# pandegroup/openmm

Hardware: NVIDIA H100
Metric: ns/day (higher is better)
Workload: dtype f32

## Files before the change

openmm_b200/csrc/engine.cu:

```cuda
#include "engine.h"
#include "../../include/b200md.h"
#include <stdexcept>
#include <algorithm>
#include <cmath>
#include <cstring>
#include <cstdlib>
#include <map>
#include <set>
#include <dlfcn.h>
#include <thread>

static std::string g_create_error;

template <class T> struct DevBuf {
    T* p = nullptr; size_t n = 0; bool owned = true;
    void attach(void* ptr, size_t count) { free(); p = (T*) ptr; n = count; owned = false; }
    void alloc(size_t count) {
        if (!owned) { if (count > n) throw std::runtime_error("window buffer too small"); return; }
        free(); n = count; if (count) CUDA_CHECK(cudaMalloc(&p, count*sizeof(T)));
    }
    void upload(const std::vector<T>& v) { if (v.size() > n) alloc(v.size()); if (!v.empty()) CUDA_CHECK(cudaMemcpy(p, v.data(), v.size()*sizeof(T), cudaMemcpyHostToDevice)); }
    void zero() { if (n) CUDA_CHECK(cudaMemset(p, 0, n*sizeof(T))); }
    void free() { if (p && owned) cudaFree(p); p = nullptr; n = 0; owned = true; }
    ~DevBuf() { free(); }
// ... 5 lines not shown
    void* lib = nullptr;
    int (*GetUniqueId)(void*) = nullptr;
    int (*CommInitRank)(void**, int, NcclUid, int) = nullptr;
    int (*AllReduce)(const void*, void*, size_t, int, int, void*, cudaStream_t) = nullptr;
    int (*AllGather)(const void*, void*, size_t, int, void*, cudaStream_t) = nullptr;
    int (*CommDestroy)(void*) = nullptr;
    const char* (*GetErrorString)(int) = nullptr;
    bool load(std::string& err) {
        if (lib) return true;
        const char* names[] = {getenv("B200MD_NCCL_LIB"), "libnccl.so.2", "libnccl.so"};
        for (const char* nm : names) { if (nm && (lib = dlopen(nm, RTLD_NOW | RTLD_GLOBAL))) break; }
        if (!lib) { err = "cannot dlopen libnccl (set B200MD_NCCL_LIB)"; return false; }
        GetUniqueId = (decltype(GetUniqueId)) dlsym(lib, "ncclGetUniqueId");
        CommInitRank = (decltype(CommInitRank)) dlsym(lib, "ncclCommInitRank");
        AllReduce = (decltype(AllReduce)) dlsym(lib, "ncclAllReduce");
        AllGather = (decltype(AllGather)) dlsym(lib, "ncclAllGather");
        CommDestroy = (decltype(CommDestroy)) dlsym(lib, "ncclCommDestroy");
        GetErrorString = (decltype(GetErrorString)) dlsym(lib, "ncclGetErrorString");
        if (!GetUniqueId || !CommInitRank || !AllReduce) { err = "libnccl lacks required symbols"; return false; }
        return true;
    }
};
static NcclApi g_nccl;
enum { NCCL_INT8 = 0, NCCL_INT64 = 4, NCCL_FLOAT32 = 7, NCCL_FLOAT64 = 8, NCCL_SUM = 0 };

struct b200md_ctx {
    int device = 0;
    int natoms = 0, npad = 0, nblocks = 0;
    bool finalized = false;
    std::string err;
    cudaStream_t stream = nullptr;
    cudaStream_t streamPme = nullptr;
    cudaStream_t streamBonded = nullptr;
    cudaEvent_t evFork = nullptr, evJoin = nullptr, evJoinBonded = nullptr;
    bool pmeOnly = false;
    bool listDirty = true;
    bool overlapPme = true;
    bool pmeBrick = true;
    int brickAtoms = 64, brickPoints = 8192;
    bool listBuilt = false;
    std::vector<double> mass, charge, sigma, epsilon;
    b200md_nonbonded_desc nbdesc{};
    bool haveNb = false;
    std::vector<int> excI, excJ; std::vector<double> excQQ, excSig, excEps;
    std::vector<int> bondI, bondJ; std::vector<double> bondR0, bondK;
    std::vector<int> angI, angJ, angK; std::vector<double> angT0, angKK;
    std::vector<int> torI, torJ, torK, torL, torN; std::vector<double> torPhase, torKK;
    std::vector<int> rbI, rbJ, rbK, rbL; std::vector<double> rbC;
    std::vector<int> cmapSize, cmapMap, cmapAtoms; std::vector<double> cmapCoeff;
    std::vector<unsigned char> bondGroup, angGroup, torGroup, rbGroup, cmapGroup;
    std::vector<int> conI, conJ; std::vector<double> conD;
    int cmFreq = 0;
    std::vector<int4> hUnitAtoms;
    double boxA[3] = {0, 0, 0}, boxB[3] = {0, 0, 0}, boxC[3] = {0, 0, 0};
    bool haveBox = false;
    bool haveOrigin = false;
    double padFrac = 0.10;
    DevBuf<float4> posq, velm, sposq[2], swrap[2], refPos, atomShift, blockCenter[2], blockHalf[2], superCenter[2], superHalf[2];
    DevBuf<float2> sigeps, ssigeps[2];
    DevBuf<double> chargeD; DevBuf<double2> sigepsD;
    DevBuf<long long> force;
    DevBuf<double> energy, cmScratch;
    DevBuf<int> molStart, molAtoms, cellOffset, sorig[2], sortedOf, cellRank, cellCount, cellFill, atomCell, tmpSorted, tileI[2], tileJ[2], tileMask[2], listCounters, counters, exclStart, exclList;
    DevBuf<unsigned int> maskPool[2];
    DevBuf<unsigned long long> stepCounter;
    DevBuf<unsigned int> blocksDone;
    bool stepStateValid = false;
// ... 58 lines not shown
static void require(bool cond, const char* msg) { if (!cond) throw std::runtime_error(msg); }
static void check_flags(b200md_ctx* c);
static void sync_velocities(b200md_ctx* c);
static void sync_positions(b200md_ctx* c);

extern "C" const char* b200md_version(void) { return "b200md 0.2 (sm_90a)"; }
extern "C" const char* b200md_last_error(const b200md_ctx* ctx) { return ctx ? ctx->err.c_str() : g_create_error.c_str(); }

extern "C" int b200md_create(b200md_ctx** out, int device, int natoms) {
    try {
        require(out != nullptr && natoms > 0, "b200md_create: bad arguments");
        int count = 0;
        cudaError_t e = cudaGetDeviceCount(&count);
        if (e != cudaSuccess || count == 0)
            throw std::runtime_error(std::string("b200md_create: no CUDA device available (") + cudaGetErrorString(e) + "); this library has no CPU fallback");
        require(device >= 0 && device < count, "b200md_create: device index out of range");
        CUDA_CHECK(cudaSetDevice(device));
        b200md_ctx* c = new b200md_ctx();
        c->device = device;
        c->natoms = natoms;
        c->npad = ((natoms + 31)/32)*32;
        c->nblocks = c->npad/32;
        CUDA_CHECK(cudaStreamCreateWithFlags(&c->stream, cudaStreamNonBlocking));
        if (getenv("B200MD_NO_OVERLAP")) c->overlapPme = false;
        if (getenv("B200MD_PME_BRICK")) c->pmeBrick = atoi(getenv("B200MD_PME_BRICK")) != 0;
        if (getenv("B200MD_PME_BRICK_POINTS")) c->brickPoints = std::max(1, atoi(getenv("B200MD_PME_BRICK_POINTS")));
        int hi = 0;
        CUDA_CHECK(cudaDeviceGetStreamPriorityRange(nullptr, &hi));
        CUDA_CHECK(cudaStreamCreateWithPriority(&c->streamPme, cudaStreamNonBlocking, hi));
        CUDA_CHECK(cudaStreamCreateWithPriority(&c->streamBonded, cudaStreamNonBlocking, hi));
        CUDA_CHECK(cudaEventCreateWithFlags(&c->evFork, cudaEventDisableTiming));
        CUDA_CHECK(cudaEventCreateWithFlags(&c->evJoin, cudaEventDisableTiming));
        CUDA_CHECK(cudaEventCreateWithFlags(&c->evJoinBonded, cudaEventDisableTiming));
        c->mass.assign(natoms, 1.0);
        c->charge.assign(natoms, 0.0); c->sigma.assign(natoms, 1.0); c->epsilon.assign(natoms, 0.0);
        const char* pf = getenv("B200MD_PAD_FRACTION");
        if (pf) c->padFrac = atof(pf);
        const char* ug = getenv("B200MD_USE_GRAPH");
        if (ug) c->useGraph = atoi(ug) != 0;
        const char* gs = getenv("B200MD_GRAPH_STEPS");
        if (gs) c->graphSteps = std::max(1, atoi(gs));
        *out = c;
        return 0;
    } catch (std::exception& e) { g_create_error = e.what(); return -1; }
}

extern "C" void b200md_destroy(b200md_ctx* ctx) {
    if (!ctx) return;
    cudaSetDevice(ctx->device);
    cudaDeviceSynchronize();
    if (ctx->stepGraph) cudaGraphExecDestroy(ctx->stepGraph);
    if (ctx->multiGraph) cudaGraphExecDestroy(ctx->multiGraph);
    for (int q = 0; q < B200MD_MAX_RANKS; q++) if (ctx->peerMapped[q]) cudaIpcCloseMemHandle(ctx->peerMapped[q]);
    if (ctx->comm && g_nccl.CommDestroy) g_nccl.CommDestroy(ctx->comm);
    if (ctx->stream) cudaStreamDestroy(ctx->stream);
    if (ctx->streamPme) cudaStreamDestroy(ctx->streamPme);
    if (ctx->streamBonded) cudaStreamDestroy(ctx->streamBonded);
    if (ctx->evFork) cudaEventDestroy(ctx->evFork);
    if (ctx->evJoin) cudaEventDestroy(ctx->evJoin);
    if (ctx->evJoinBonded) cudaEventDestroy(ctx->evJoinBonded);
    char* window = ctx->window;
    delete ctx;
    if (window) cudaFree(window);
}

extern "C" int b200md_set_masses(b200md_ctx* ctx, const double* mass) {
    API_BEGIN(ctx)
    require(!ctx->finalized, "set_masses after finalize");
    ctx->mass.assign(mass, mass + ctx->natoms);
    API_END(ctx)
}

extern "C" int b200md_set_nonbonded(b200md_ctx* ctx, const b200md_nonbonded_desc* d, const double* q, const double* sig, const double* eps) {
    API_BEGIN(ctx)
    require(!ctx->finalized, "set_nonbonded after finalize");
    require(d->method != B200MD_NB_EWALD && d->method != B200MD_NB_LJPME, "nonbonded method not supported by the B200 platform (only NoCutoff, CutoffNonPeriodic, CutoffPeriodic, PME)");
    ctx->nbdesc = *d;
    ctx->haveNb = true;
    ctx->charge.assign(q, q + ctx->natoms);
    ctx->sigma.assign(sig, sig + ctx->natoms);
    ctx->epsilon.assign(eps, eps + ctx->natoms);
    ctx->dispersionCoefficient = d->dispersion_coefficient;
    API_END(ctx)
}

extern "C" int b200md_set_exceptions(b200md_ctx* ctx, int n, const int* p1, const int* p2, const double* qq, const double* sig, const double* eps) {
    API_BEGIN(ctx)
    require(!ctx->finalized, "set_exceptions after finalize");
    ctx->excI.assign(p1, p1+n); ctx->excJ.assign(p2, p2+n);
    ctx->excQQ.assign(qq, qq+n); ctx->excSig.assign(sig, sig+n); ctx->excEps.assign(eps, eps+n);
    API_END(ctx)
}
extern "C" int b200md_set_bonds(b200md_ctx* ctx, int n, const int* p1, const int* p2, const double* len, const double* k) {
// ... 1206 lines not shown
    PmeDev p = c->pme;
    p.brickAtoms = (c->pmeBrick && c->world == 1 && !c->pmeOnly && c->listBuilt) ? c->brickAtoms : 0;
    p.brickPoints = c->brickPoints;
    return p;
}

static int enqueue_forces(b200md_ctx* c, int terms, bool energy, bool forcesAlreadyZero = false, bool inStep = false, unsigned int groupMask = 0xffffffffu) {
    int launches = 0;
    cudaStream_t s = c->stream;
    if (!forcesAlreadyZero) CUDA_CHECK(cudaMemsetAsync(c->force.p, 0, sizeof(long long)*3*c->npad, s));
    if (energy) CUDA_CHECK(cudaMemsetAsync(c->energy.p, 0, sizeof(double)*B200MD_NUM_ENERGY, s));
    bool direct = (terms & B200MD_TERM_NB_DIRECT) && c->haveNb;
    bool recip = (terms & B200MD_TERM_NB_RECIP) && c->haveNb && c->nb.method == B200MD_NB_PME;
    const bool split = role_split(c);
    const int pmeRank = c->world - 1;
    NbDev nbSave = c->nb;
    if (split) {
        if (c->rank == pmeRank) direct = false; else recip = false;
        c->nb = role_nb(c);
    }
    struct Restore { b200md_ctx* c; NbDev saved; ~Restore() { c->nb = saved; } } restore{c, nbSave};
    const bool p2p = c->p2p;
    const bool fork = direct && recip && c->overlapPme && !(c->world > 1 && c->comm && !p2p);
    cudaStream_t sp = fork ? c->streamPme : s;
    if (p2p && !direct) { launch_pos_wait(c->nb, c->cd, s); launches++; }
    const PmeDev pme = pme_for_launch(c);
    const bool forkAfterList = fork && direct && pme.brickAtoms > 0;
    auto launch_recip = [&]() {
        if (fork) {
            CUDA_CHECK(cudaEventRecord(c->evFork, s));
            CUDA_CHECK(cudaStreamWaitEvent(sp, c->evFork, 0));
        }
        if (recip) {
            launch_pme_spread(c->nb, pme, c->cd, sp); launches++;
            if (p2p) { launch_grid_push(c->pme, c->cd, sp); launches++; }
            else if (c->world > 1 && c->comm && !split) {
                int rc = g_nccl.AllReduce(c->gridFixed.p, c->gridFixed.p, (size_t) c->pme.nx*c->pme.ny*c->pme.nz, NCCL_INT64, NCCL_SUM, c->comm, sp);
                if (rc != 0) throw std::runtime_error("ncclAllReduce(grid) failed");
            }
            launch_pme_fft_conv(c->nb, c->pme, c->cd, energy && (split || p2p || c->rank == 0), fft_beside_tiles(c), sp); launches += pme_fft_launch_count(c->pme);
            launch_pme_gather(c->nb, pme, c->cd, sp); launches++;
        }
        if (fork) CUDA_CHECK(cudaEventRecord(c->evJoin, sp));
    };
    if (!forkAfterList) launch_recip();
    if (direct) {
        launch_check_displacement(c->nb, c->cd, s); launches++;
        launch_list_build(c->nb, s); launches += LIST_BUILD_LAUNCHES;
    }
    int bterms = terms & (B200MD_TERM_BONDS | B200MD_TERM_ANGLES | B200MD_TERM_TORSIONS | B200MD_TERM_RB_TORSIONS | B200MD_TERM_CMAP);
    if (c->haveNb) bterms |= terms & B200MD_TERM_NB_DIRECT;
    const int nbonded = c->bd.nbonds + c->bd.nangles + c->bd.ntorsions + c->bd.nrb + c->bd.ncmap + c->bd.nexc;
    const bool bonded = bterms && nbonded > 0 && !(split && c->rank == pmeRank);
    auto launch_bonded_terms = [&](cudaStream_t sb) { BondedDev bd = c->bd; bd.groupMask = groupMask; launch_bonded(c->nb, bd, bterms, energy, sb); launches++; };
    const bool forkBonded = forkAfterList && bonded;
    if (forkAfterList) launch_recip();
    if (forkBonded) {
        CUDA_CHECK(cudaStreamWaitEvent(c->streamBonded, c->evFork, 0));
        launch_bonded_terms(c->streamBonded);
        CUDA_CHECK(cudaEventRecord(c->evJoinBonded, c->streamBonded));
    }
    if (direct) { launch_pair(c->nb, energy, s); launches++; }
    if (bonded && !forkBonded) launch_bonded_terms(s);
    const bool pushEarly = p2p && fork;
    if (pushEarly) { launch_force_push(c->nb, c->cd, s); launches++; }
    if (fork) CUDA_CHECK(cudaStreamWaitEvent(s, c->evJoin, 0));
    if (forkBonded) CUDA_CHECK(cudaStreamWaitEvent(s, c->evJoinBonded, 0));
    if (p2p) {
        if (!pushEarly) { launch_force_push(c->nb, c->cd, s); launches++; }
        if (!inStep) { launch_force_total(c->nb, c->cd, s); launches += 2; }
    }
    if (c->world > 1 && c->comm) {
        int rc = 0;
        if (!p2p) rc = g_nccl.AllReduce(c->force.p, c->force.p, (size_t) 3*c->npad, NCCL_INT64, NCCL_SUM, c->comm, s);
        if (rc != 0) throw std::runtime_error("ncclAllReduce(force) failed");
        if (energy) {
            rc = g_nccl.AllReduce(c->energy.p, c->energy.p, B200MD_NUM_ENERGY, NCCL_FLOAT64, NCCL_SUM, c->comm, s);
            if (rc != 0) throw std::runtime_error("ncclAllReduce(energy) failed");
// ... 421 lines not shown
```

openmm_b200/csrc/engine.h:

```cpp
#pragma once
#include <cuda_runtime.h>
#include <stdint.h>
#include <stdexcept>
#include <string>
#include <vector>

#define B200MD_TILE 32
#define B200MD_PME_ORDER 5
#define B200MD_FORCE_SCALE 4294967296.0
#define B200MD_ONE_4PI_EPS0 138.93545764438198
#define B200MD_BOLTZ 0.00831446261815324
#define B200MD_MAX_RADIX 16
#define B200MD_MAX_FFT_STAGES 8

#define CUDA_CHECK(x) do { cudaError_t e_ = (x); if (e_ != cudaSuccess) throw std::runtime_error(std::string(#x) + ": " + cudaGetErrorString(e_)); } while (0)

template <typename... P, typename... A>
inline void launch_high(void (*kernel)(P...), dim3 grid, dim3 block, size_t smem, cudaStream_t s, A... args) {
    static const int hi = [] { int lo = 0, h = 0; cudaDeviceGetStreamPriorityRange(&lo, &h); return h; }();
    cudaLaunchAttribute at[1];
    at[0].id = cudaLaunchAttributePriority;
    at[0].val.priority = hi;
    cudaLaunchConfig_t cfg = {};
    cfg.gridDim = grid; cfg.blockDim = block; cfg.dynamicSmemBytes = smem; cfg.stream = s;
// ... 322 lines not shown
__device__ __forceinline__ float3 gauss3(unsigned int seed, int atom, unsigned long long step) {
    uint4 r = philox(make_uint4((unsigned int) atom, (unsigned int) step, (unsigned int) (step >> 32), 0x5eed5eedu), make_uint2(seed, 0xb200b200u));
    const float u1 = ((r.x >> 8) + 1u)*(1.0f/16777216.0f);
    const float u2 = (r.y >> 8)*(1.0f/16777216.0f);
    const float u3 = ((r.z >> 8) + 1u)*(1.0f/16777216.0f);
    const float u4 = (r.w >> 8)*(1.0f/16777216.0f);
    const float m1 = sqrtf(-2.0f*logf(u1)), m2 = sqrtf(-2.0f*logf(u3));
    float s1, c1, s2, c2;
    sincospif(2.0f*u2, &s1, &c1);
    sincospif(2.0f*u4, &s2, &c2);
    (void) s2;
    return make_float3(m1*c1, m1*s1, m2*c2);
}

#endif

struct ScaleDev {
    int nmol;
    const int* molStart;
    const int* molAtoms;
    double a[3], b[3], c[3];
    double s[3];
};

void launch_check_displacement(const NbDev& nb, const CommDev& cd, cudaStream_t s);
const int LIST_BUILD_LAUNCHES = 2;
void launch_list_build(const NbDev& nb, cudaStream_t s);
void launch_pair(const NbDev& nb, bool energy, cudaStream_t s);
void pair_set_carveout(size_t fftSmem, size_t brickSmem);
void launch_count_pairs(const NbDev& nb, cudaStream_t s);
int choose_pme_sms(int reserve, unsigned long long mask[4]);

void launch_pme_eterm(const NbDev& nb, const PmeDev& pme, cudaStream_t s);
void launch_pme_spread(const NbDev& nb, const PmeDev& pme, const CommDev& cd, cudaStream_t s);
void launch_pme_fft_conv(const NbDev& nb, const PmeDev& pme, const CommDev& cd, bool energy, bool besideTiles, cudaStream_t s);
void launch_pme_gather(const NbDev& nb, const PmeDev& pme, const CommDev& cd, cudaStream_t s);
void pme_brick_setup(int maxSmem);
void launch_grid_push(const PmeDev& pme, const CommDev& cd, cudaStream_t s);
void launch_fft3d_r2c(const PmeDev& pme, cudaStream_t s);
void launch_fft3d_c2r(const PmeDev& pme, cudaStream_t s);
size_t fft_plane_smem_bytes(int ny, int nz);
size_t fft_line_smem_bytes(int nx);
bool fft_make_radices(int n, int* radix, int* nstages);
int pme_fft_launch_count(const PmeDev& pme);
void fft_set_compact(int on);
size_t fft_cta_smem_bytes(const PmeDev& pme);
bool fft_slab_path(const PmeDev& pme);

void launch_bonded(const NbDev& nb, const BondedDev& bd, int terms, bool energy, cudaStream_t s);

void launch_integrate(const NbDev& nb, const UnitDev& units, const IntegDev& integ, const CommDev& cd, cudaStream_t s);
void launch_force_push(const NbDev& nb, const CommDev& cd, cudaStream_t s);
void launch_pos_push(const NbDev& nb, const CommDev& cd, const IntegDev& in, cudaStream_t s);
bool pos_push_available();
void launch_force_total(const NbDev& nb, const CommDev& cd, cudaStream_t s);
void launch_vel_push(const NbDev& nb, const CommDev& cd, cudaStream_t s);
void launch_pos_wait(const NbDev& nb, const CommDev& cd, cudaStream_t s);
void launch_constrain_positions(const NbDev& nb, const UnitDev& units, double tol, cudaStream_t s);
void launch_constrain_velocities(const NbDev& nb, const UnitDev& units, double tol, cudaStream_t s);
void launch_kinetic_energy(const NbDev& nb, const UnitDev& units, const IntegDev& integ, double shiftDt, cudaStream_t s);
void launch_remove_cm(const NbDev& nb, double* scratch, cudaStream_t s);
void launch_scale_molecules(const NbDev& nb, const ScaleDev& sc, cudaStream_t s);
void launch_ccma_step(const NbDev& nb, const CcmaDev& cc, const IntegDev& in, cudaStream_t s);
void launch_ccma_apply(const NbDev& nb, const CcmaDev& cc, bool velocities, double tol, cudaStream_t s);
void launch_ccma_kinetic(const NbDev& nb, const CcmaDev& cc, double shiftDt, double tol, cudaStream_t s);
void launch_cm_prime(const NbDev& nb, const IntegDev& integ, const CommDev& cd, cudaStream_t s);
```

openmm_b200/csrc/integrate.cu:

```cuda
#include "engine.h"
#include <algorithm>
#include "../../include/b200md.h"

template <class R> struct V3 { R x, y, z; };
template <class R> __device__ __forceinline__ V3<R> operator+(V3<R> a, V3<R> b) { return {a.x+b.x, a.y+b.y, a.z+b.z}; }
template <class R> __device__ __forceinline__ V3<R> operator-(V3<R> a, V3<R> b) { return {a.x-b.x, a.y-b.y, a.z-b.z}; }
template <class R> __device__ __forceinline__ V3<R> operator*(V3<R> a, R s) { return {a.x*s, a.y*s, a.z*s}; }
template <class R> __device__ __forceinline__ R dot(V3<R> a, V3<R> b) { return a.x*b.x + a.y*b.y + a.z*b.z; }

template <class R>
__device__ void settle_positions(const V3<R>* x, V3<R>* d, const R* m, R dist1, R dist2) {
    const V3<R> xp0 = d[0], xp1 = d[1], xp2 = d[2];
    const R xb0 = x[1].x-x[0].x, yb0 = x[1].y-x[0].y, zb0 = x[1].z-x[0].z;
    const R xc0 = x[2].x-x[0].x, yc0 = x[2].y-x[0].y, zc0 = x[2].z-x[0].z;
    const R invTotalMass = R(1)/(m[0]+m[1]+m[2]);
    const R xcom = (xp0.x*m[0] + (xb0+xp1.x)*m[1] + (xc0+xp2.x)*m[2])*invTotalMass;
    const R ycom = (xp0.y*m[0] + (yb0+xp1.y)*m[1] + (yc0+xp2.y)*m[2])*invTotalMass;
    const R zcom = (xp0.z*m[0] + (zb0+xp1.z)*m[1] + (zc0+xp2.z)*m[2])*invTotalMass;
    const R xa1 = xp0.x - xcom, ya1 = xp0.y - ycom, za1 = xp0.z - zcom;
    const R xb1 = xb0 + xp1.x - xcom, yb1 = yb0 + xp1.y - ycom, zb1 = zb0 + xp1.z - zcom;
    const R xc1 = xc0 + xp2.x - xcom, yc1 = yc0 + xp2.y - ycom, zc1 = zc0 + xp2.z - zcom;
    const R xaksZd = yb0*zc0 - zb0*yc0, yaksZd = zb0*xc0 - xb0*zc0, zaksZd = xb0*yc0 - yb0*xc0;
    const R xaksXd = ya1*zaksZd - za1*yaksZd, yaksXd = za1*xaksZd - xa1*zaksZd, zaksXd = xa1*yaksZd - ya1*xaksZd;
    const R xaksYd = yaksZd*zaksXd - zaksZd*yaksXd, yaksYd = zaksZd*xaksXd - xaksZd*zaksXd, zaksYd = xaksZd*yaksXd - yaksZd*xaksXd;
// ... 131 lines not shown
        U.n = k+1;
        const R4<R> p = load_pos<R>(nb, a);
        const R4<R> v = vel_array<R>(nb)[a];
        U.x[k] = {p.x, p.y, p.z};
        U.v[k] = {v.x, v.y, v.z};
        U.invM[k] = v.w;
        U.m[k] = (v.w > R(0)) ? R(1)/v.w : R(0);
        if (wantForce) {
            long long fx = nb.force[a], fy = nb.force[a + nb.npad], fz = nb.force[a + 2*nb.npad];
            if (cd != nullptr && cd->world > 1) {
                const long long* in = (const long long*) (cd->peer[cd->rank] + cd->offFinbox);
                for (int q = 0; q < cd->world; q++) if (q != cd->rank) {
                    const long long* iq = in + (size_t) q*3*nb.npad;
                    fx += iq[a]; fy += iq[a + nb.npad]; fz += iq[a + 2*nb.npad];
                }
            }
            U.f[k] = {fixed_to_real<R>(fx), fixed_to_real<R>(fy), fixed_to_real<R>(fz)};
        }
    }
    return true;
}

template <class R>
__device__ __forceinline__ void constrain_pos(const Unit<R>& U, V3<R>* d, R tol) {
    if (U.type == 1) settle_positions(U.x, d, U.m, U.prm.x, U.prm.y);
    else if (U.type == 2) { const R dist[3] = {U.prm.x, U.prm.y, U.prm.z}; shake_positions(U.x, d, U.invM, dist, U.n-1, tol); }
}
template <class R>
__device__ __forceinline__ void constrain_vel(const Unit<R>& U, V3<R>* v, R tol) {
    if (U.type == 1) settle_velocities(U.x, v, U.m);
    else if (U.type == 2) shake_velocities(U.x, v, U.invM, U.n-1, tol);
}

template <int KIND, class R>
__global__ void __launch_bounds__(128, sizeof(R) == 8 ? 1 : 0) k_integrate(NbDev nb, UnitDev un, IntegDev in, CommDev cd) {
    const bool multi = cd.world > 1;
    const bool useInbox = multi && in.fused;
    const unsigned long long E = multi ? *cd.epoch + 1ull : 0ull;
    if (useInbox) comm_wait(cd, CH_FORCE, E);
    const int u = (multi ? cd.unitLo[cd.rank] : 0) + blockIdx.x*blockDim.x + threadIdx.x;
    const bool active = u < (multi ? cd.unitLo[cd.rank + 1] : un.nunits);
    const unsigned long long step = *in.stepCounter;
    const IntegR<R> ic = integ_r<R>(in);
    Unit<R> U;
    U.n = 0;
    V3<R> d[4];
    const R invDt = R(1)/ic.dt;
    const bool cmFused = in.fused && in.cmEveryStep;
    V3<R> vcm = {R(0), R(0), R(0)};
    if (cmFused) {
        double c[4];
        if (multi) {
            const double* t = (const double*) (cd.peer[cd.rank] + cd.offCm) + 4*(step % 3ull);
            c[0] = c[1] = c[2] = c[3] = 0.0;
            for (int q = 0; q < cd.world; q++) for (int k = 0; k < 4; k++) c[k] += t[q*12 + k];
        }
        else { const double* t = in.cmScratch + 4*(step % 3ull); c[0] = t[0]; c[1] = t[1]; c[2] = t[2]; c[3] = t[3]; }
        const double im = (c[3] > 0.0) ? 1.0/c[3] : 0.0;
        vcm = {(R) (c[0]*im), (R) (c[1]*im), (R) (c[2]*im)};
    }
    if (active) {
    load_unit(nb, un, u, U, true, useInbox ? &cd : nullptr);
    if (in.fused) {
        _Pragma("unroll") for (int k = 0; k < 4; k++) if (k < U.n) {
            const int a = U.atom[k];
            nb.force[a] = 0; nb.force[a + nb.npad] = 0; nb.force[a + 2*nb.npad] = 0;
            if (U.invM[k] > R(0)) U.v[k] = U.v[k] - vcm;
        }
    }
    if (KIND == B200MD_INT_LANGEVIN_MIDDLE) {
        _Pragma("unroll") for (int k = 0; k < 4; k++) if (k < U.n) U.v[k] = U.v[k] + U.f[k]*(ic.dt*U.invM[k]);
        constrain_vel(U, U.v, ic.tol);
        V3<R> du[4];
        _Pragma("unroll") for (int k = 0; k < 4; k++) if (k < U.n) {
            d[k] = U.v[k]*(R(0.5)*ic.dt);
            if (U.invM[k] > R(0)) {
                const float3 g = gauss3(in.seed, U.atom[k], step);
                const R ns = ic.noisescale*sqrt_r(ic.kT*U.invM[k]);
                U.v[k] = U.v[k]*ic.vscale + V3<R>{g.x, g.y, g.z}*ns;
            }
            d[k] = d[k] + U.v[k]*(R(0.5)*ic.dt);
            if (U.invM[k] == R(0)) d[k] = {R(0), R(0), R(0)};
            du[k] = d[k];
        }
        constrain_pos(U, d, ic.tol);
        _Pragma("unroll") for (int k = 0; k < 4; k++) if (k < U.n) U.v[k] = U.v[k] + (d[k] - du[k])*invDt;
    }
    else {
        _Pragma("unroll") for (int k = 0; k < 4; k++) if (k < U.n) {
            V3<R> vn;
            if (KIND == B200MD_INT_LANGEVIN) {
                vn = U.v[k]*ic.vscale + U.f[k]*(ic.fscale*U.invM[k]);
                if (U.invM[k] > R(0) && ic.noisescale > R(0)) {
                    const float3 g = gauss3(in.seed, U.atom[k], step);
                    vn = vn + V3<R>{g.x, g.y, g.z}*(ic.noisescale*sqrt_r(U.invM[k]));
                }
            }
            else
                vn = U.v[k] + U.f[k]*(ic.dt*U.invM[k]);
            if (U.invM[k] == R(0)) vn = U.v[k];
            d[k] = (U.invM[k] == R(0)) ? V3<R>{R(0), R(0), R(0)} : vn*ic.dt;
        }
        constrain_pos(U, d, ic.tol);
        _Pragma("unroll") for (int k = 0; k < 4; k++) if (k < U.n) if (U.invM[k] > R(0)) U.v[k] = d[k]*invDt;
    }
    _Pragma("unroll") for (int k = 0; k < 4; k++) if (k < U.n) {
        const int a = U.atom[k];
        store_pos<R>(nb, a, U.x[k].x + d[k].x, U.x[k].y + d[k].y, U.x[k].z + d[k].z);
        vel_array<R>(nb)[a] = make_r4(U.v[k].x, U.v[k].y, U.v[k].z, U.invM[k]);
        if (multi && !cd.posByPush) {
            const float4 pn = nb.posq[a];
            for (int k = 1; k < cd.world; k++) {
                const int q = (cd.rank + k) % cd.world;
                ((float4*) (cd.peer[q] + cd.offPosq))[a] = pn;
            }
        }
    }
    }
    if (!in.fused && !(multi && !cd.posByPush)) return;
    if (cmFused) {
        double px = 0, py = 0, pz = 0, m = 0;
        _Pragma("unroll") for (int k = 0; k < 4; k++) if (k < U.n && U.invM[k] > R(0)) {
            const double mk = U.m[k];
            px += mk*U.v[k].x; py += mk*U.v[k].y; pz += mk*U.v[k].z; m += mk;
        }
        for (int off = 16; off > 0; off >>= 1) {
            px += __shfl_xor_sync(0xffffffffu, px, off); py += __shfl_xor_sync(0xffffffffu, py, off);
            pz += __shfl_xor_sync(0xffffffffu, pz, off); m += __shfl_xor_sync(0xffffffffu, m, off);
        }
        __shared__ double red[4][4];
        if ((threadIdx.x & 31) == 0) { red[threadIdx.x >> 5][0] = px; red[threadIdx.x >> 5][1] = py; red[threadIdx.x >> 5][2] = pz; red[threadIdx.x >> 5][3] = m; }
        __syncthreads();
        if (threadIdx.x < 4) {
            double t = 0;
            for (int w = 0; w < (int) (blockDim.x >> 5); w++) t += red[w][threadIdx.x];
            atomicAdd(&in.cmScratch[4*((step + 1ull) % 3ull) + threadIdx.x], t);
            if (blockIdx.x == 0) in.cmScratch[4*((step + 2ull) % 3ull) + threadIdx.x] = 0.0;
        }
    }
    if (multi && !cd.posByPush) {
        const bool lastBlock = comm_arrive(cd, CH_POS, gridDim.x);
        if (lastBlock && threadIdx.x == 0) {
            if (cmFused) {
                const double* mine = in.cmScratch + 4*((step + 1ull) % 3ull);
                for (int q = 0; q < cd.world; q++) {
                    double* t = (double*) (cd.peer[q] + cd.offCm) + cd.rank*12 + 4*((step + 1ull) % 3ull);
                    for (int k = 0; k < 4; k++) t[k] = ((volatile const double*) mine)[k];
                }
            }
            comm_publish(cd, CH_POS, E);
            *cd.posNeed = E;
            *cd.epoch = E;
            *in.stepCounter = step + 1ull;
        }
        return;
    }
    __shared__ int last;
    __syncthreads();
    if (threadIdx.x == 0) {
        __threadfence();
        last = (atomicAdd(in.blocksDone, 1u) == gridDim.x - 1);
    }
    __syncthreads();
    if (last && threadIdx.x == 0) {
        *in.blocksDone = 0u;
        *in.stepCounter = step + 1ull;
    }
}
// ... 7 lines not shown
    const int a = blockIdx.x*blockDim.x + threadIdx.x;
    double px = 0, py = 0, pz = 0, m = 0;
    if (a < nb.natoms) {
        const R4<R> v = vel_array<R>(nb)[a];
        if (v.w > R(0)) { m = 1.0/v.w; px = m*v.x; py = m*v.y; pz = m*v.z; }
    }
    for (int off = 16; off > 0; off >>= 1) {
        px += __shfl_xor_sync(0xffffffffu, px, off); py += __shfl_xor_sync(0xffffffffu, py, off);
        pz += __shfl_xor_sync(0xffffffffu, pz, off); m += __shfl_xor_sync(0xffffffffu, m, off);
    }
    __shared__ double red[8][4];
    if ((threadIdx.x & 31) == 0) { red[threadIdx.x >> 5][0] = px; red[threadIdx.x >> 5][1] = py; red[threadIdx.x >> 5][2] = pz; red[threadIdx.x >> 5][3] = m; }
    __syncthreads();
    if (threadIdx.x < 4) {
        double t = 0;
        for (int w = 0; w < 8; w++) t += red[w][threadIdx.x];
        atomicAdd(&c[threadIdx.x], t);
    }
}

void launch_cm_prime(const NbDev& nb, const IntegDev& integ, const CommDev& cd, cudaStream_t s) {
    cudaMemsetAsync(integ.cmScratch, 0, 12*sizeof(double), s);
    double* table = integ.cmScratch;
    if (cd.world > 1) {
        table = (double*) (cd.peer[cd.rank] + cd.offCm);
        cudaMemsetAsync(table, 0, (size_t) B200MD_MAX_RANKS*12*sizeof(double), s);
    }
    if (nb.velmD) k_cm_prime<double><<<(nb.natoms + 255)/256, 256, 0, s>>>(nb, integ, table);
    else k_cm_prime<float><<<(nb.natoms + 255)/256, 256, 0, s>>>(nb, integ, table);
}

template <int KIND>
static void launch_integrate_kind(int grid, const NbDev& nb, const UnitDev& units, const IntegDev& integ, const CommDev& cd, cudaStream_t s) {
    if (nb.velmD) k_integrate<KIND, double><<<grid, 64, 0, s>>>(nb, units, integ, cd);
    else k_integrate<KIND, float><<<grid, 64, 0, s>>>(nb, units, integ, cd);
}

void launch_integrate(const NbDev& nb, const UnitDev& units, const IntegDev& integ, const CommDev& cd, cudaStream_t s) {
    const int n = cd.world > 1 ? cd.unitLo[cd.rank + 1] - cd.unitLo[cd.rank] : units.nunits;
    const int grid = std::max(1, (n + 63)/64);
    if (integ.kind == B200MD_INT_VERLET) launch_integrate_kind<B200MD_INT_VERLET>(grid, nb, units, integ, cd, s);
    else if (integ.kind == B200MD_INT_LANGEVIN) launch_integrate_kind<B200MD_INT_LANGEVIN>(grid, nb, units, integ, cd, s);
    else launch_integrate_kind<B200MD_INT_LANGEVIN_MIDDLE>(grid, nb, units, integ, cd, s);
    if (!integ.fused && (cd.world <= 1 || cd.posByPush)) k_step_advance<<<1, 1, 0, s>>>(integ);
    if (cd.world > 1 && cd.posByPush) launch_pos_push(nb, cd, integ, s);
}

template <class R>
__global__ void __launch_bounds__(128) k_constrain_positions(NbDev nb, UnitDev un, R tol) {
    const int u = blockIdx.x*blockDim.x + threadIdx.x;
    if (u >= un.nunits) return;
    Unit<R> U;
    load_unit(nb, un, u, U, false);
    if (U.type == 0) return;
    V3<R> d[4] = {{0, 0, 0}, {0, 0, 0}, {0, 0, 0}, {0, 0, 0}};
    constrain_pos(U, d, tol);
    _Pragma("unroll") for (int k = 0; k < 4; k++) if (k < U.n) {
        const int a = U.atom[k];
        const R4<R> p = load_pos<R>(nb, a);
        store_pos<R>(nb, a, p.x + d[k].x, p.y + d[k].y, p.z + d[k].z);
    }
}

template <class R>
__global__ void __launch_bounds__(128) k_constrain_velocities(NbDev nb, UnitDev un, R tol) {
    const int u = blockIdx.x*blockDim.x + threadIdx.x;
    if (u >= un.nunits) return;
    Unit<R> U;
    load_unit(nb, un, u, U, false);
    if (U.type == 0) return;
    constrain_vel(U, U.v, tol);
    _Pragma("unroll") for (int k = 0; k < 4; k++) if (k < U.n) vel_array<R>(nb)[U.atom[k]] = make_r4(U.v[k].x, U.v[k].y, U.v[k].z, U.invM[k]);
}
// ... 126 lines not shown
```

openmm_b200/csrc/pme.cu:

```cuda
#include "engine.h"
#include <algorithm>
#include <climits>
#include <stdexcept>

#define ORDER B200MD_PME_ORDER

typedef double wreal;
__device__ __forceinline__ void bspline(wreal dr, wreal* data, wreal* ddata) {
    data[ORDER-1] = 0.f;
    data[1] = dr;
    data[0] = 1.f - dr;
#pragma unroll
    for (int k = 3; k < ORDER; k++) {
        const wreal div = 1.f/(k - 1.f);
        data[k-1] = div*dr*data[k-2];
#pragma unroll
        for (int l = 1; l < k-1; l++)
            data[k-l-1] = div*((dr + l)*data[k-l-2] + (k - l - dr)*data[k-l-1]);
        data[0] = div*(1.f - dr)*data[0];
    }
    ddata[0] = -data[0];
#pragma unroll
    for (int k = 1; k < ORDER; k++) ddata[k] = data[k-1] - data[k];
    const wreal div = 1.f/(ORDER - 1);
// ... 229 lines not shown
__global__ void k_pme_eterm(NbDev nb, PmeDev pme) {
    const size_t total = (size_t) pme.nx*pme.ny*pme.nzc;
    const size_t i = (size_t) blockIdx.x*blockDim.x + threadIdx.x;
    if (i >= total) return;
    const int kz = (int) (i % pme.nzc);
    const int ky = (int) ((i / pme.nzc) % pme.ny);
    const int kx = (int) (i / ((size_t) pme.nzc*pme.ny));
    if (kx == 0 && ky == 0 && kz == 0) { pme.eterm[i] = 0; return; }
    const double* R = nb.box.recip;
    const double mx = (kx < (pme.nx+1)/2) ? kx : kx - pme.nx;
    const double my = (ky < (pme.ny+1)/2) ? ky : ky - pme.ny;
    const double mz = (kz < (pme.nz+1)/2) ? kz : kz - pme.nz;
    const double mhx = mx*R[0];
    const double mhy = mx*R[3] + my*R[4];
    const double mhz = mx*R[6] + my*R[7] + mz*R[8];
    const double m2 = mhx*mhx + mhy*mhy + mhz*mhz;
    const double pi = 3.14159265358979323846;
    const double factor = pi*pi/(pme.alpha*pme.alpha);
    const double denom = m2*pi*nb.box.volume*pme.moduli[0][kx]*pme.moduli[1][ky]*pme.moduli[2][kz];
    pme.eterm[i] = (real) (exp(-factor*m2)/denom);
}

void launch_pme_eterm(const NbDev& nb, const PmeDev& pme, cudaStream_t s) {
    size_t total = (size_t) pme.nx*pme.ny*pme.nzc;
    k_pme_eterm<<<(unsigned) ((total + 255)/256), 256, 0, s>>>(nb, pme);
}

void pme_brick_setup(int maxSmem) {
    cudaFuncAttributes fa;
    CUDA_CHECK(cudaFuncGetAttributes(&fa, k_pme_spread_brick));
    CUDA_CHECK(cudaFuncSetAttribute(k_pme_spread_brick, cudaFuncAttributeMaxDynamicSharedMemorySize, maxSmem - (int) fa.sharedSizeBytes));
}

void launch_pme_spread(const NbDev& nb, const PmeDev& pme, const CommDev& cd, cudaStream_t s) {
    cudaMemsetAsync(pme.gridFixed, 0, sizeof(long long)*(size_t) pme.nx*pme.ny*pme.nz, s);
    if (pme.brickAtoms > 0) {
        launch_high(k_pme_spread_brick, (nb.npad + pme.brickAtoms - 1)/pme.brickAtoms, 256, sizeof(long long)*pme.brickPoints, s, nb, pme);
        return;
    }
    const int per = cd.world > 1 ? cd.atomLo[cd.rank + 1] - cd.atomLo[cd.rank] : (nb.natoms + nb.world - 1)/nb.world;
    launch_high(k_pme_spread, std::max(1, (per*8 + 127)/128), 128, 0, s, nb, pme, cd);
}

void launch_pme_gather(const NbDev& nb, const PmeDev& pme, const CommDev& cd, cudaStream_t s) {
    const int per = cd.world > 1 ? cd.atomLo[cd.rank + 1] - cd.atomLo[cd.rank] : (nb.natoms + nb.world - 1)/nb.world;
    launch_high(k_pme_gather, std::max(1, (per + 127)/128), 128, 0, s, nb, pme, cd);
}
```

Baseline: 1374.

## Spread integrator across four lanes per unit and overlap PME grid clear with list build

The integrator kernel now assigns one thread per atom (four lanes per constraint unit) instead of one thread per unit. Lanes exchange positions and displacements with warp shuffles only when a constraint solve is needed, which raises memory-level parallelism and removes per-thread serial loops over atoms. Separately, when PME spreading is forked after the neighbor list build, the grid memset is issued early on the PME stream so it overlaps the list build. The cost is redundant constraint solves on every lane of a unit, plus extra shuffle and shared-memory work for the centre-of-mass reduction.

After: 1419 (median of 6 runs). 3.3% higher.

```diff
diff --git a/openmm_b200/csrc/engine.cu b/openmm_b200/csrc/engine.cu
--- a/openmm_b200/csrc/engine.cu
+++ b/openmm_b200/csrc/engine.cu
@@ -61,7 +61,7 @@
     cudaStream_t stream = nullptr;
     cudaStream_t streamPme = nullptr;
     cudaStream_t streamBonded = nullptr;
-    cudaEvent_t evFork = nullptr, evJoin = nullptr, evJoinBonded = nullptr;
+    cudaEvent_t evFork = nullptr, evJoin = nullptr, evJoinBonded = nullptr, evForkGrid = nullptr;
     bool pmeOnly = false;
     bool listDirty = true;
     bool overlapPme = true;
@@ -186,6 +186,7 @@
         CUDA_CHECK(cudaEventCreateWithFlags(&c->evFork, cudaEventDisableTiming));
         CUDA_CHECK(cudaEventCreateWithFlags(&c->evJoin, cudaEventDisableTiming));
         CUDA_CHECK(cudaEventCreateWithFlags(&c->evJoinBonded, cudaEventDisableTiming));
+        CUDA_CHECK(cudaEventCreateWithFlags(&c->evForkGrid, cudaEventDisableTiming));
         c->mass.assign(natoms, 1.0);
         c->charge.assign(natoms, 0.0); c->sigma.assign(natoms, 1.0); c->epsilon.assign(natoms, 0.0);
         const char* pf = getenv("B200MD_PAD_FRACTION");
@@ -213,6 +214,7 @@
     if (ctx->evFork) cudaEventDestroy(ctx->evFork);
     if (ctx->evJoin) cudaEventDestroy(ctx->evJoin);
     if (ctx->evJoinBonded) cudaEventDestroy(ctx->evJoinBonded);
+    if (ctx->evForkGrid) cudaEventDestroy(ctx->evForkGrid);
     char* window = ctx->window;
     delete ctx;
     if (window) cudaFree(window);
@@ -1485,7 +1487,7 @@
             CUDA_CHECK(cudaStreamWaitEvent(sp, c->evFork, 0));
         }
         if (recip) {
-            launch_pme_spread(c->nb, pme, c->cd, sp); launches++;
+            launch_pme_spread(c->nb, pme, c->cd, sp, !forkAfterList); launches++;
             if (p2p) { launch_grid_push(c->pme, c->cd, sp); launches++; }
             else if (c->world > 1 && c->comm && !split) {
                 int rc = g_nccl.AllReduce(c->gridFixed.p, c->gridFixed.p, (size_t) c->pme.nx*c->pme.ny*c->pme.nz, NCCL_INT64, NCCL_SUM, c->comm, sp);
@@ -1497,6 +1499,11 @@
         if (fork) CUDA_CHECK(cudaEventRecord(c->evJoin, sp));
     };
     if (!forkAfterList) launch_recip();
+    if (forkAfterList && recip) {
+        CUDA_CHECK(cudaEventRecord(c->evForkGrid, s));
+        CUDA_CHECK(cudaStreamWaitEvent(sp, c->evForkGrid, 0));
+        CUDA_CHECK(cudaMemsetAsync(pme.gridFixed, 0, sizeof(long long)*(size_t) pme.nx*pme.ny*pme.nz, sp));
+    }
     if (direct) {
         launch_check_displacement(c->nb, c->cd, s); launches++;
         launch_list_build(c->nb, s); launches += LIST_BUILD_LAUNCHES;
diff --git a/openmm_b200/csrc/engine.h b/openmm_b200/csrc/engine.h
--- a/openmm_b200/csrc/engine.h
+++ b/openmm_b200/csrc/engine.h
@@ -378,7 +378,7 @@
 int choose_pme_sms(int reserve, unsigned long long mask[4]);
 
 void launch_pme_eterm(const NbDev& nb, const PmeDev& pme, cudaStream_t s);
-void launch_pme_spread(const NbDev& nb, const PmeDev& pme, const CommDev& cd, cudaStream_t s);
+void launch_pme_spread(const NbDev& nb, const PmeDev& pme, const CommDev& cd, cudaStream_t s, bool zeroGrid = true);
 void launch_pme_fft_conv(const NbDev& nb, const PmeDev& pme, const CommDev& cd, bool energy, bool besideTiles, cudaStream_t s);
 void launch_pme_gather(const NbDev& nb, const PmeDev& pme, const CommDev& cd, cudaStream_t s);
 void pme_brick_setup(int maxSmem);
diff --git a/openmm_b200/csrc/integrate.cu b/openmm_b200/csrc/integrate.cu
--- a/openmm_b200/csrc/integrate.cu
+++ b/openmm_b200/csrc/integrate.cu
@@ -187,19 +187,35 @@
     else if (U.type == 2) shake_velocities(U.x, v, U.invM, U.n-1, tol);
 }
 
+constexpr int INTEG_LANES = 4;
+constexpr int INTEG_UNITS = 64;
+constexpr int INTEG_THREADS = INTEG_LANES*INTEG_UNITS;
+
+__device__ __forceinline__ float shfl_r(float x, int src) { return __shfl_sync(0xffffffffu, x, src); }
+__device__ __forceinline__ double shfl_r(double x, int src) { return __shfl_sync(0xffffffffu, x, src); }
+template <class R>
+__device__ __forceinline__ V3<R> shfl_v3(V3<R> a, int src) { return {shfl_r(a.x, src), shfl_r(a.y, src), shfl_r(a.z, src)}; }
+
+template <class T>
+__device__ __forceinline__ T pick(const T* w, int k) {
+    T r = w[0];
+    _Pragma("unroll") for (int j = 1; j < 4; j++) if (k == j) r = w[j];
+    return r;
+}
+
 template <int KIND, class R>
-__global__ void __launch_bounds__(128, sizeof(R) == 8 ? 1 : 0) k_integrate(NbDev nb, UnitDev un, IntegDev in, CommDev cd) {
+__global__ void __launch_bounds__(INTEG_THREADS, 1) k_integrate(NbDev nb, UnitDev un, IntegDev in, CommDev cd) {
     const bool multi = cd.world > 1;
     const bool useInbox = multi && in.fused;
     const unsigned long long E = multi ? *cd.epoch + 1ull : 0ull;
     if (useInbox) comm_wait(cd, CH_FORCE, E);
-    const int u = (multi ? cd.unitLo[cd.rank] : 0) + blockIdx.x*blockDim.x + threadIdx.x;
+    const int ka = threadIdx.x & (INTEG_LANES - 1);
+    const int g = threadIdx.x & 31 & ~(INTEG_LANES - 1);
+    const int ub = threadIdx.x / INTEG_LANES;
+    const int u = (multi ? cd.unitLo[cd.rank] : 0) + blockIdx.x*INTEG_UNITS + ub;
     const bool active = u < (multi ? cd.unitLo[cd.rank + 1] : un.nunits);
     const unsigned long long step = *in.stepCounter;
     const IntegR<R> ic = integ_r<R>(in);
-    Unit<R> U;
-    U.n = 0;
-    V3<R> d[4];
     const R invDt = R(1)/ic.dt;
     const bool cmFused = in.fused && in.cmEveryStep;
     V3<R> vcm = {R(0), R(0), R(0)};
@@ -214,55 +230,100 @@
         const double im = (c[3] > 0.0) ? 1.0/c[3] : 0.0;
         vcm = {(R) (c[0]*im), (R) (c[1]*im), (R) (c[2]*im)};
     }
+    Unit<R> U;
+    U.n = 0; U.type = 0;
+    int a = -1;
     if (active) {
-    load_unit(nb, un, u, U, true, useInbox ? &cd : nullptr);
-    if (in.fused) {
-        _Pragma("unroll") for (int k = 0; k < 4; k++) if (k < U.n) {
-            const int a = U.atom[k];
+        const int4 at = un.unitAtoms[u];
+        U.n = at.w >= 0 ? 4 : at.z >= 0 ? 3 : at.y >= 0 ? 2 : at.x >= 0 ? 1 : 0;
+        a = ka == 0 ? at.x : ka == 1 ? at.y : ka == 2 ? at.z : at.w;
+        U.type = un.unitType[u];
+        U.prm = unit_params<R>(un, u);
+    }
+    const bool own = a >= 0;
+    V3<R> x = {R(0), R(0), R(0)}, v = x, f = x, d = x;
+    R invM = R(0), m = R(0);
+    if (own) {
+        const R4<R> p = load_pos<R>(nb, a);
+        const R4<R> vm = vel_array<R>(nb)[a];
+        x = {p.x, p.y, p.z};
+        v = {vm.x, vm.y, vm.z};
+        invM = vm.w;
+        m = (vm.w > R(0)) ? R(1)/vm.w : R(0);
+        long long fx = nb.force[a], fy = nb.force[a + nb.npad], fz = nb.force[a + 2*nb.npad];
+        if (useInbox) {
+            const long long* inbox = (const long long*) (cd.peer[cd.rank] + cd.offFinbox);
+            for (int q = 0; q < cd.world; q++) if (q != cd.rank) {
+                const long long* iq = inbox + (size_t) q*3*nb.npad;
+                fx += iq[a]; fy += iq[a + nb.npad]; fz += iq[a + 2*nb.npad];
+            }
+        }
+        f = {fixed_to_real<R>(fx), fixed_to_real<R>(fy), fixed_to_real<R>(fz)};
+        if (in.fused) {
             nb.force[a] = 0; nb.force[a + nb.npad] = 0; nb.force[a + 2*nb.npad] = 0;
-            if (U.invM[k] > R(0)) U.v[k] = U.v[k] - vcm;
-        }
-    }
+            if (invM > R(0)) v = v - vcm;
+        }
+    }
+    const bool solve = __any_sync(0xffffffffu, U.type != 0);
+    if (solve) {
+        _Pragma("unroll") for (int j = 0; j < 4; j++) {
+            U.x[j] = shfl_v3(x, g + j);
+            U.invM[j] = shfl_r(invM, g + j);
+            U.m[j] = shfl_r(m, g + j);
+        }
+    }
+    V3<R> uw[4];
     if (KIND == B200MD_INT_LANGEVIN_MIDDLE) {
-        _Pragma("unroll") for (int k = 0; k < 4; k++) if (k < U.n) U.v[k] = U.v[k] + U.f[k]*(ic.dt*U.invM[k]);
-        constrain_vel(U, U.v, ic.tol);
-        V3<R> du[4];
-        _Pragma("unroll") for (int k = 0; k < 4; k++) if (k < U.n) {
-            d[k] = U.v[k]*(R(0.5)*ic.dt);
-            if (U.invM[k] > R(0)) {
-                const float3 g = gauss3(in.seed, U.atom[k], step);
-                const R ns = ic.noisescale*sqrt_r(ic.kT*U.invM[k]);
-                U.v[k] = U.v[k]*ic.vscale + V3<R>{g.x, g.y, g.z}*ns;
-            }
-            d[k] = d[k] + U.v[k]*(R(0.5)*ic.dt);
-            if (U.invM[k] == R(0)) d[k] = {R(0), R(0), R(0)};
-            du[k] = d[k];
-        }
-        constrain_pos(U, d, ic.tol);
-        _Pragma("unroll") for (int k = 0; k < 4; k++) if (k < U.n) U.v[k] = U.v[k] + (d[k] - du[k])*invDt;
+        if (own) v = v + f*(ic.dt*invM);
+        if (solve) {
+            _Pragma("unroll") for (int j = 0; j < 4; j++) uw[j] = shfl_v3(v, g + j);
+            constrain_vel(U, uw, ic.tol);
+            v = pick(uw, ka);
+        }
+        V3<R> du = d;
+        if (own) {
+            d = v*(R(0.5)*ic.dt);
+            if (invM > R(0)) {
+                const float3 gn = gauss3(in.seed, a, step);
+                const R ns = ic.noisescale*sqrt_r(ic.kT*invM);
+                v = v*ic.vscale + V3<R>{gn.x, gn.y, gn.z}*ns;
+            }
+            d = d + v*(R(0.5)*ic.dt);
+            if (invM == R(0)) d = {R(0), R(0), R(0)};
+            du = d;
+        }
+        if (solve) {
+            _Pragma("unroll") for (int j = 0; j < 4; j++) uw[j] = shfl_v3(d, g + j);
+            constrain_pos(U, uw, ic.tol);
+            d = pick(uw, ka);
+        }
+        if (own) v = v + (d - du)*invDt;
     }
     else {
-        _Pragma("unroll") for (int k = 0; k < 4; k++) if (k < U.n) {
+        if (own) {
             V3<R> vn;
             if (KIND == B200MD_INT_LANGEVIN) {
-                vn = U.v[k]*ic.vscale + U.f[k]*(ic.fscale*U.invM[k]);
-                if (U.invM[k] > R(0) && ic.noisescale > R(0)) {
-                    const float3 g = gauss3(in.seed, U.atom[k], step);
-                    vn = vn + V3<R>{g.x, g.y, g.z}*(ic.noisescale*sqrt_r(U.invM[k]));
+                vn = v*ic.vscale + f*(ic.fscale*invM);
+                if (invM > R(0) && ic.noisescale > R(0)) {
+                    const float3 gn = gauss3(in.seed, a, step);
+                    vn = vn + V3<R>{gn.x, gn.y, gn.z}*(ic.noisescale*sqrt_r(invM));
                 }
             }
             else
-                vn = U.v[k] + U.f[k]*(ic.dt*U.invM[k]);
-            if (U.invM[k] == R(0)) vn = U.v[k];
-            d[k] = (U.invM[k] == R(0)) ? V3<R>{R(0), R(0), R(0)} : vn*ic.dt;
-        }
-        constrain_pos(U, d, ic.tol);
-        _Pragma("unroll") for (int k = 0; k < 4; k++) if (k < U.n) if (U.invM[k] > R(0)) U.v[k] = d[k]*invDt;
-    }
-    _Pragma("unroll") for (int k = 0; k < 4; k++) if (k < U.n) {
-        const int a = U.atom[k];
-        store_pos<R>(nb, a, U.x[k].x + d[k].x, U.x[k].y + d[k].y, U.x[k].z + d[k].z);
-        vel_array<R>(nb)[a] = make_r4(U.v[k].x, U.v[k].y, U.v[k].z, U.invM[k]);
+                vn = v + f*(ic.dt*invM);
+            if (invM == R(0)) vn = v;
+            d = (invM == R(0)) ? V3<R>{R(0), R(0), R(0)} : vn*ic.dt;
+        }
+        if (solve) {
+            _Pragma("unroll") for (int j = 0; j < 4; j++) uw[j] = shfl_v3(d, g + j);
+            constrain_pos(U, uw, ic.tol);
+            d = pick(uw, ka);
+        }
+        if (own && invM > R(0)) v = d*invDt;
+    }
+    if (own) {
+        store_pos<R>(nb, a, x.x + d.x, x.y + d.y, x.z + d.z);
+        vel_array<R>(nb)[a] = make_r4(v.x, v.y, v.z, invM);
         if (multi && !cd.posByPush) {
             const float4 pn = nb.posq[a];
             for (int k = 1; k < cd.world; k++) {
@@ -271,24 +332,32 @@
             }
         }
     }
-    }
     if (!in.fused && !(multi && !cd.posByPush)) return;
     if (cmFused) {
-        double px = 0, py = 0, pz = 0, m = 0;
-        _Pragma("unroll") for (int k = 0; k < 4; k++) if (k < U.n && U.invM[k] > R(0)) {
-            const double mk = U.m[k];
-            px += mk*U.v[k].x; py += mk*U.v[k].y; pz += mk*U.v[k].z; m += mk;
-        }
-        for (int off = 16; off > 0; off >>= 1) {
-            px += __shfl_xor_sync(0xffffffffu, px, off); py += __shfl_xor_sync(0xffffffffu, py, off);
-            pz += __shfl_xor_sync(0xffffffffu, pz, off); m += __shfl_xor_sync(0xffffffffu, m, off);
-        }
-        __shared__ double red[4][4];
-        if ((threadIdx.x & 31) == 0) { red[threadIdx.x >> 5][0] = px; red[threadIdx.x >> 5][1] = py; red[threadIdx.x >> 5][2] = pz; red[threadIdx.x >> 5][3] = m; }
+        const bool mine = own && invM > R(0);
+        double px = 0, py = 0, pz = 0, pm = 0;
+        _Pragma("unroll") for (int j = 0; j < 4; j++) {
+            const int cj = __shfl_sync(0xffffffffu, (int) mine, g + j);
+            const double mk = shfl_r((double) m, g + j);
+            const V3<R> vj = shfl_v3(v, g + j);
+            if (cj) { px += mk*vj.x; py += mk*vj.y; pz += mk*vj.z; pm += mk; }
+        }
+        __shared__ double unitP[INTEG_UNITS][4];
+        if (ka == 0) { unitP[ub][0] = px; unitP[ub][1] = py; unitP[ub][2] = pz; unitP[ub][3] = pm; }
+        __shared__ double red[INTEG_UNITS/32][4];
+        __syncthreads();
+        if (threadIdx.x < INTEG_UNITS) {
+            px = unitP[threadIdx.x][0]; py = unitP[threadIdx.x][1]; pz = unitP[threadIdx.x][2]; pm = unitP[threadIdx.x][3];
+            for (int off = 16; off > 0; off >>= 1) {
+                px += __shfl_xor_sync(0xffffffffu, px, off); py += __shfl_xor_sync(0xffffffffu, py, off);
+                pz += __shfl_xor_sync(0xffffffffu, pz, off); pm += __shfl_xor_sync(0xffffffffu, pm, off);
+            }
+            if ((threadIdx.x & 31) == 0) { red[threadIdx.x >> 5][0] = px; red[threadIdx.x >> 5][1] = py; red[threadIdx.x >> 5][2] = pz; red[threadIdx.x >> 5][3] = pm; }
+        }
         __syncthreads();
         if (threadIdx.x < 4) {
             double t = 0;
-            for (int w = 0; w < (int) (blockDim.x >> 5); w++) t += red[w][threadIdx.x];
+            for (int w = 0; w < INTEG_UNITS/32; w++) t += red[w][threadIdx.x];
             atomicAdd(&in.cmScratch[4*((step + 1ull) % 3ull) + threadIdx.x], t);
             if (blockIdx.x == 0) in.cmScratch[4*((step + 2ull) % 3ull) + threadIdx.x] = 0.0;
         }
@@ -362,13 +431,13 @@
 
 template <int KIND>
 static void launch_integrate_kind(int grid, const NbDev& nb, const UnitDev& units, const IntegDev& integ, const CommDev& cd, cudaStream_t s) {
-    if (nb.velmD) k_integrate<KIND, double><<<grid, 64, 0, s>>>(nb, units, integ, cd);
-    else k_integrate<KIND, float><<<grid, 64, 0, s>>>(nb, units, integ, cd);
+    if (nb.velmD) k_integrate<KIND, double><<<grid, INTEG_THREADS, 0, s>>>(nb, units, integ, cd);
+    else k_integrate<KIND, float><<<grid, INTEG_THREADS, 0, s>>>(nb, units, integ, cd);
 }
 
 void launch_integrate(const NbDev& nb, const UnitDev& units, const IntegDev& integ, const CommDev& cd, cudaStream_t s) {
     const int n = cd.world > 1 ? cd.unitLo[cd.rank + 1] - cd.unitLo[cd.rank] : units.nunits;
-    const int grid = std::max(1, (n + 63)/64);
+    const int grid = std::max(1, (n + INTEG_UNITS - 1)/INTEG_UNITS);
     if (integ.kind == B200MD_INT_VERLET) launch_integrate_kind<B200MD_INT_VERLET>(grid, nb, units, integ, cd, s);
     else if (integ.kind == B200MD_INT_LANGEVIN) launch_integrate_kind<B200MD_INT_LANGEVIN>(grid, nb, units, integ, cd, s);
     else launch_integrate_kind<B200MD_INT_LANGEVIN_MIDDLE>(grid, nb, units, integ, cd, s);
diff --git a/openmm_b200/csrc/pme.cu b/openmm_b200/csrc/pme.cu
--- a/openmm_b200/csrc/pme.cu
+++ b/openmm_b200/csrc/pme.cu
@@ -285,8 +285,8 @@
     CUDA_CHECK(cudaFuncSetAttribute(k_pme_spread_brick, cudaFuncAttributeMaxDynamicSharedMemorySize, maxSmem - (int) fa.sharedSizeBytes));
 }
 
-void launch_pme_spread(const NbDev& nb, const PmeDev& pme, const CommDev& cd, cudaStream_t s) {
-    cudaMemsetAsync(pme.gridFixed, 0, sizeof(long long)*(size_t) pme.nx*pme.ny*pme.nz, s);
+void launch_pme_spread(const NbDev& nb, const PmeDev& pme, const CommDev& cd, cudaStream_t s, bool zeroGrid) {
+    if (zeroGrid) cudaMemsetAsync(pme.gridFixed, 0, sizeof(long long)*(size_t) pme.nx*pme.ny*pme.nz, s);
     if (pme.brickAtoms > 0) {
         launch_high(k_pme_spread_brick, (nb.npad + pme.brickAtoms - 1)/pme.brickAtoms, 256, sizeof(long long)*pme.brickPoints, s, nb, pme);
         return;
```
